# parrot-tts/Parrot-TTS

Measured on AMD Instinct MI355X. Metric: audio samples/sec (16 kHz; see config.note) + RTF, 256-unit batch-64 per GPU, higher is better.
Workload: dtype f32 (f16x3 split products)

## Files before the change

### include/parrot_hip_debug.h

```cpp
#ifndef PARROT_HIP_DEBUG_H
#define PARROT_HIP_DEBUG_H

#include "parrot_hip.h"

#ifdef __cplusplus
extern "C" {
#endif

int parrot_selftest(void* stream);
int parrot_conv_num_tile_cfgs(void);

int parrot_set_default_precision(int32_t prec);
int parrot_set_fused_resblocks(int32_t mode);
int parrot_set_tte_merge(int32_t on);
int parrot_debug_copy(const float* src, float* dst, size_t n, void* stream);
int parrot_debug_mfma_ceiling(int32_t shape, int32_t constant_data, double* tflops_out);
int parrot_prof_begin(void);
int parrot_prof_begin_row(int32_t row);
int parrot_prof_end(double* out, int32_t n_cfg);

int parrot_voc_debug_absmax(parrot_voc_t*, float* dst_dev);
int parrot_tte_debug_stages(parrot_tte_t*, float* const* enc_ptrs, float* const* dec_ptrs);
size_t parrot_debug_attention_workspace_bytes(int32_t B, int32_t T, int32_t H, int32_t core);
int parrot_debug_attention(const float* qkv, const uint8_t* valid, float* ctx, int32_t B, int32_t T, int32_t H, int32_t hd, int32_t core,
                           void* ws, size_t ws_bytes, void* stream);
int parrot_debug_layernorm(const float* x, const float* gamma, const float* beta, float* y, int32_t B, int32_t C, int32_t T,
                           int32_t relu_in, void* stream);
#define PARROT_DEBUG_MAX_DIM (1 << 20)
int parrot_debug_durations(const float* ld_raw, const uint8_t* src_valid, const int32_t* src_len, int32_t B, int32_t S, float* log_dur,
                           int64_t* dur, int32_t* cum, int32_t* out_len, int32_t* status, void* stream);
// ... 60 lines not shown
```

### parrot_tts_amd/_lib.py

```python
from __future__ import annotations

import ctypes as C
import os

HERE = os.path.dirname(os.path.abspath(__file__))
LIB_PATH = os.environ.get("PARROT_HIP_LIB") or os.path.join(HERE, "libparrot_hip.so")

MAX_STAGES, MAX_KERNELS, MAX_DIL = 8, 4, 4
ABI_VERSION = 7
c_float_p = C.POINTER(C.c_float)


class ParrotHipError(RuntimeError):
    def __init__(self, code: int, msg: str):
        super().__init__(f"libparrot_hip error {code}: {msg}")
        self.code = code


class ConvDesc(C.Structure):
    _fields_ = [("c_in", C.c_int32), ("c_out", C.c_int32), ("k", C.c_int32), ("dilation", C.c_int32),
                ("padding", C.c_int32), ("transposed", C.c_int32), ("stride", C.c_int32), ("pre_act", C.c_int32),
                ("pre_slope", C.c_float), ("act", C.c_int32), ("tile_cfg", C.c_int32), ("precision", C.c_int32)]


# ... 100 lines not shown

vp, i32, sz, f32 = C.c_void_p, C.c_int32, C.c_size_t, C.c_float
SIGNATURES = {
    "parrot_abi_version": (C.c_int, []),
    "parrot_last_error": (C.c_char_p, []),
    "parrot_selftest": (C.c_int, [vp]),
    "parrot_set_default_precision": (C.c_int, [i32]),
    "parrot_set_fused_resblocks": (C.c_int, [i32]),
    "parrot_set_tte_merge": (C.c_int, [i32]),
    "parrot_conv_create": (C.c_int, [C.POINTER(vp), C.POINTER(ConvDesc), c_float_p, c_float_p]),
    "parrot_conv_destroy": (None, [vp]),
    "parrot_conv_run": (C.c_int, [vp, vp, vp, vp, i32, i32, i32, f32, vp]),
    "parrot_conv_out_len": (C.c_int, [vp, i32]),
    "parrot_conv_num_tile_cfgs": (C.c_int, []),
    "parrot_debug_copy": (C.c_int, [vp, vp, sz, vp]),
    "parrot_debug_mfma_ceiling": (C.c_int, [i32, i32, C.POINTER(C.c_double)]),
    "parrot_prof_begin": (C.c_int, []),
    "parrot_prof_begin_row": (C.c_int, [i32]),
    "parrot_prof_end": (C.c_int, [C.POINTER(C.c_double), i32]),
    "parrot_voc_create": (C.c_int, [C.POINTER(vp), C.POINTER(VocCfg), C.POINTER(VocWeights)]),
    "parrot_voc_create_ex": (C.c_int, [C.POINTER(vp), C.POINTER(VocCfg), C.POINTER(VocWeights), i32, i32]),
    "parrot_voc_destroy": (None, [vp]),
    "parrot_voc_precision": (C.c_int, [vp]),
    "parrot_voc_debug_absmax": (C.c_int, [vp, vp]),
    "parrot_voc_workspace_bytes": (sz, [vp, i32, i32]),
    "parrot_voc_forward": (C.c_int, [vp, vp, vp, vp, i32, i32, vp, C.POINTER(vp), vp, sz, vp]),
    "parrot_voc_forward_feats": (C.c_int, [vp, vp, vp, vp, i32, vp, i32, i32, vp, C.POINTER(vp), vp, sz, vp]),
    "parrot_voc_chunked_workspace_bytes": (sz, [vp, i32, i32, i32]),
    "parrot_voc_forward_chunked": (C.c_int, [vp, vp, vp, vp, i32, i32, i32, i32, vp, vp, sz, vp]),
    "parrot_voc_check": (C.c_int, [vp, vp]),
# ... 131 lines not shown
```

### parrot_tts_amd/csrc/conv_mfma.h

```cpp
#pragma once
#include <hip/hip_runtime.h>
#include <stdint.h>
#include <algorithm>

#include "conv_consts.h"
#include "div_uniform.h"

namespace parrot {

__host__ __device__ __forceinline__ int row_true_len(int n, int mul, int add) { return n > 0 ? n * mul + add : 0; }

struct DynLdsOnce {
    bool done[64] = {};
};
inline hipError_t ensure_dyn_lds(DynLdsOnce& st, const void* kern, size_t lds) {
    int dev = 0;
    hipError_t e = hipGetDevice(&dev);
    if (e != hipSuccess) return e;
    const bool tracked = dev >= 0 && dev < 64;
    if (tracked && st.done[dev]) return hipSuccess;
    e = hipFuncSetAttribute(kern, hipFuncAttributeMaxDynamicSharedMemorySize, (int)lds);
    if (e == hipSuccess && tracked) st.done[dev] = true;
    return e;
}
// ... 23 lines not shown
    int act;
    int epi;
    float div;
    int u;
    int tiles_n;
    long x_bstride;
    long y_bstride;
    long res_bstride;
    int groups;
    int Mg;
    int u_inv16;
    const int32_t* row_len;
    int row_len_mul;
    int row_len_add;
    int fold_res;
    int lean;
    int n_cus;
    int epi16;
    float acc_scale;
    float out_scale;
    const void* xplane;
    void* yplane;
    long xplane_bstride;
    long yplane_bstride;
    float yplane_slope;
    int plane_only;
};

__device__ __forceinline__ float apply_act(float v, int act) { return (act == ACT_RELU && v < 0.f) ? 0.f : v; }

// ... 146 lines not shown
#pragma unroll
                    for (int q = 0; q < 8; ++q) yv[q] = yb[off[q] < 0 ? 0 : off[q]];
                }
                float v[8];
#pragma unroll
                for (int q = 0; q < 8; ++q) v[q] = yv[q] + (fmaxf(acc[mt][nt][g * 8 + q], act_lo) + rv[q]);
                if (do_div) div_rows(dv, v);
#pragma unroll
                for (int q = 0; q < 8; ++q)
                    if (off[q] >= 0) yb[off[q]] = v[q];
            }
        }
    }
}

struct RowTile {
    __amdgpu_buffer_rsrc_t rsrc;
};
__device__ __forceinline__ RowTile row_tile(const float* base, int rows, int row_elems) {
    const size_t a = reinterpret_cast<size_t>(base);
    const unsigned lo = __builtin_amdgcn_readfirstlane((unsigned)a), hi = __builtin_amdgcn_readfirstlane((unsigned)(a >> 32));
    RowTile t;
    t.rsrc = __builtin_amdgcn_make_buffer_rsrc(reinterpret_cast<void*>(((size_t)hi << 32) | lo), 0,
                                               __builtin_amdgcn_readfirstlane(rows * row_elems * 4), 0x00020000);
    return t;
}
__device__ __forceinline__ float row_tile_load(const RowTile& t, int voff, int soff) {
    return __builtin_bit_cast(float, __builtin_amdgcn_raw_buffer_load_b32(t.rsrc, voff, soff, 0));
}
__device__ __forceinline__ void row_tile_store(const RowTile& t, float v, int voff, int soff) {
// ... 272 lines not shown
```

### parrot_tts_amd/csrc/conv_split.h

```cpp
#pragma once
#include <cstdlib>
#include <type_traits>

#include "conv_mfma.h"

namespace parrot {

typedef short s16x8 __attribute__((ext_vector_type(8)));
typedef __bf16 bf16x8 __attribute__((ext_vector_type(8)));
typedef _Float16 f16x8 __attribute__((ext_vector_type(8)));

typedef __bf16 bf16x2 __attribute__((ext_vector_type(2)));
typedef _Float16 f16x2 __attribute__((ext_vector_type(2)));
typedef float f32x2 __attribute__((ext_vector_type(2)));
__device__ __forceinline__ unsigned pk_bf16(float x0, float x1) {
    const f32x2 v = {x0, x1};
    return __builtin_bit_cast(unsigned, __builtin_convertvector(v, bf16x2));
}
__device__ __forceinline__ unsigned pk_f16(float x0, float x1) {
    const f32x2 v = {x0, x1};
    return __builtin_bit_cast(unsigned, __builtin_convertvector(v, f16x2));
}
__device__ __forceinline__ float max_nc(float a, float b) {
    float r;
// ... 63 lines not shown
}
template <class SCH>
__device__ __forceinline__ float pre_scale(float v, float slope) {
    if constexpr (SCH::XS != 1.f) return max_nc(v * SCH::XS, v * (SCH::XS * slope));
    else return max_nc(v, v * slope);
}

template <int N, class F>
__device__ __forceinline__ void static_for(F&& f) {
    if constexpr (N > 0) {
        static_for<N - 1>(f);
        f(std::integral_constant<int, N - 1>{});
    }
}

template <class SCH, int WAVES_M, int WAVES_N, int WM, int WN, int MINW, int K, int SUBS = 1, bool LEAN = false>
__global__ __launch_bounds__(WAVES_M* WAVES_N * 64, MINW) void conv_split_kernel(const ConvParams p) {
    static_assert(SUBS == 1 || K == 1, "sub-slab staging: 1x1 convs only (no halo)");
    constexpr int NPC = SCH::NP, NTERM = SCH::NT;
    constexpr int NW = WAVES_M * WAVES_N, NT = NW * 64;
    constexpr int BM = WAVES_M * WM * 32;
    constexpr int BN = WAVES_N * WN * 32;
    constexpr int COLS = BN + ((SUBS > 1 && K == 1) ? 0 : CONV_HALO);
    constexpr int PIECE_BYTES = COLS * 32;
    constexpr int SUB_BYTES = NPC * PIECE_BYTES;
    constexpr int BUF_BYTES = SUBS * SUB_BYTES;
    constexpr int LIVE = SUBS * COLS * 2;
    constexpr int ITEMS = (LIVE + NT - 1) / NT;
    constexpr int KS = K * SUBS;
    constexpr int STEP_BYTES = NPC * 1024;

    extern __shared__ __attribute__((aligned(16))) char smem_raw[];

    const int tid = threadIdx.x;
    const int lane = tid & 63;
    const int wave = __builtin_amdgcn_readfirstlane(tid >> 6);
    const int wm = wave / WAVES_N;
    const int wn = wave % WAVES_N;
    const int half = lane >> 5;
    const int l31 = lane & 31;

    const int n_mb = (p.M + BM - 1) / BM;
    const int n_tiles = p.tiles_n * p.B, tpx = (n_tiles + 7) >> 3;
    const int xcd = blockIdx.x & 7, seq = blockIdx.x >> 3;
// ... 70 lines not shown
    for (int mt = 0; mt < WM; ++mt)
        abase[mt] = __builtin_amdgcn_readfirstlane((int)((mblock * (BM / 32) + wm * WM + mt) * p.n_it * STEP_BYTES));
    const unsigned lane16 = lane * 16;
    const int nsup = p.nchunks / SUBS;
    const int colbase = wn * WN * 32 + l31;
    auto load_b = [&](s16x8 (&bb)[WN][NPC], const char* __restrict__ xs, int tap) {
        const int col = colbase + tap * p.dil;
        const int off = col * 32 + ((half ^ ((col >> 3) & 1)) * 16);
#pragma unroll
        for (int nt = 0; nt < WN; ++nt)
#pragma unroll
            for (int pc = 0; pc < NPC; ++pc) bb[nt][pc] = *reinterpret_cast<const s16x8*>(xs + pc * PIECE_BYTES + nt * 1024 + off);
    };
    constexpr int TM = WM * WN, NMF = NTERM * TM;
    if constexpr (K > 0) {
        s16x8 A[2][WM][NPC], Bv[2][WN][NPC];
        auto load_a_piece = [&](s16x8 (&a)[WM][NPC], int pc, int soff) {
#pragma unroll
            for (int mt = 0; mt < WM; ++mt)
                a[mt][pc] = __builtin_bit_cast(s16x8, __builtin_amdgcn_raw_buffer_load_b128(wrsrc, lane16 + pc * 1024, abase[mt] + soff, 0));
        };
        auto next_chunk = [&](int q) { return (q + 1 == nsup) ? 0 : q + 1; };
        int cc = 0, cn = next_chunk(0);
#pragma unroll
        for (int pc = 0; pc < NPC; ++pc) {
            load_a_piece(A[0], pc, cc * KS * STEP_BYTES);
            load_a_piece(A[1], pc, (KS > 1 ? cc * KS + 1 : cn * KS) * STEP_BYTES);
        }
        load_slab(0);
        store_slab(0);
        __syncthreads();
        auto chunk = [&](auto par, int c) __attribute__((always_inline)) {
            constexpr int PAR = decltype(par)::value;
            const char* __restrict__ xs = smem_raw + (c & 1) * BUF_BYTES;
            const int cn2 = next_chunk(cn);
            load_slab(cn);
            load_b(Bv[PAR], xs, 0);
#pragma unroll
            for (int j = 0; j < KS; ++j) {
                const int cur = (PAR + j) & 1;
                const int tq = (j + 2 < KS) ? cc : (KS == 1 ? cn2 : cn);
                const int tj = (j + 2 < KS) ? j + 2 : (KS == 1 ? 0 : j + 2 - KS);
                const int soff = (tq * KS + tj) * STEP_BYTES;
                if (j + 1 < KS) load_b(Bv[cur ^ 1], xs + ((j + 1) / K) * SUB_BYTES, (j + 1) % K);
#pragma unroll
                for (int t = 0; t < NTERM; ++t) {
#pragma unroll
                    for (int mt = 0; mt < WM; ++mt)
#pragma unroll
                        for (int nt = 0; nt < WN; ++nt)
                            acc[mt][nt] = mfma32<SCH>(A[cur][mt][SCH::pa(t)], Bv[cur][nt][SCH::pb(t)], acc[mt][nt]);
#pragma unroll
                    for (int pc = 0; pc < NPC; ++pc)
                        if (t == SCH::last_a(pc)) load_a_piece(A[cur], pc, soff);
                }
            }
            constexpr int DS_START = (NPC >= 2) ? (SCH::last_a(NPC - 1) + 1) * TM - 1 + WM : 0;
            constexpr int SLAB_START = (NPC >= 2) ? (SCH::last_a(1) + 1) * TM - 1 + WM : 0;
            constexpr int SLAB_SLOTS = (NMF - SLAB_START) > 0 ? (NMF - SLAB_START) : 1, SLAB_PER = (ITEMS * 8 + SLAB_SLOTS - 1) / SLAB_SLOTS;
#pragma unroll
            for (int i = 0; i < NPC * WN; ++i) __builtin_amdgcn_sched_group_barrier(0x100, 1, 0);
#pragma unroll
            for (int j = 0; j < KS; ++j) {
                int ds_left = (j + 1 < KS) ? NPC * WN : 0, slab_left = (j == 0) ? ITEMS * 8 : 0;
#pragma unroll
                for (int m = 0; m < NMF; ++m) {
                    __builtin_amdgcn_sched_group_barrier(0x008, 1, 0);
#pragma unroll
                    for (int pc = NPC - 1; pc >= 1; --pc)
                        if (m >= (SCH::last_a(pc) + 1) * TM - 1 && m < (SCH::last_a(pc) + 1) * TM - 1 + WM) __builtin_amdgcn_sched_group_barrier(0x020, 1, 0);
                    if (m >= DS_START && ds_left > 0) {
                        __builtin_amdgcn_sched_group_barrier(0x100, 1, 0);
                        --ds_left;
                    }
                    if (m >= SLAB_START)
#pragma unroll
// ... 70 lines not shown
                xs = smem_raw + (c & 1) * BUF_BYTES;
                cc = cn;
                cn = (cc + 1 == p.nchunks) ? 0 : cc + 1;
                j = 0;
            } else {
                ++j;
            }
        };
        const int total = p.nchunks * p.k;
        for (int st = 0; st < total; st += 2) {
            step(a0, b0, a1, b1);
            if (st + 1 < total) step(a1, b1, a0, b0);
        }
    }
    if constexpr (LEAN) conv_epilogue_lean<WM, WN>(p, acc, b, m_wave, n_wave, half, l31);
    else conv_epilogue<WM, WN>(p, acc, b, m_wave, n_wave, half, l31);
}

template <class SCH, int WAVES_M, int WAVES_N, int WM, int WN, int MINW, int K, int SUBS = 1, bool LEAN = false>
inline hipError_t launch_conv_split_t(const ConvParams& p, dim3 grid, hipStream_t s) {
    constexpr int BN = WAVES_N * WN * 32;
    const size_t lds = (size_t)2 * SUBS * SCH::NP * (BN + ((SUBS > 1 && K == 1) ? 0 : CONV_HALO)) * 32;
    auto kern = conv_split_kernel<SCH, WAVES_M, WAVES_N, WM, WN, MINW, K, SUBS, LEAN>;
    static DynLdsOnce lds_once;
    {
        hipError_t e = ensure_dyn_lds(lds_once, reinterpret_cast<const void*>(kern), (size_t)lds);
        if (e != hipSuccess) return e;
    }
    hipLaunchKernelGGL(kern, grid, dim3(WAVES_M * WAVES_N * 64), lds, s, p);
    return hipGetLastError();
}

inline void split_tile(int variant, int& bm, int& bn) {
    if (variant == 2) { bm = 128; bn = 64; return; }
    if (variant == 3) { bm = 32; bn = 512; return; }
    bm = (variant & 1) ? 64 : 128;
    bn = (variant & 1) ? 256 : 128;
}
inline unsigned split_grid(const ConvParams& p, int bm) {
    const unsigned tiles = (unsigned)p.tiles_n * p.B, n_mb = (p.M + bm - 1) / bm;
    return (tiles + 7) / 8 * 8 * n_mb;
}
template <class SCH>
inline hipError_t launch_conv_split_s(int variant, const ConvParams& p, hipStream_t s) {
    int bm, bn;
    split_tile(variant, bm, bn);
    dim3 grid(split_grid(p, bm));
    if (variant == 3) return p.k == 3 ? launch_conv_split_t<SCH, 1, 4, 1, 4, 2, 3>(p, grid, s) : launch_conv_split_t<SCH, 1, 4, 1, 4, 2, 0>(p, grid, s);
    const bool lean = conv_lean_ok(p);
    if constexpr (SCH::ID == SchF16x3::ID) if (variant == 2) {
        if (p.k == 1 && p.nchunks % 4 == 0)
            return lean ? launch_conv_split_t<SCH, 4, 1, 1, 2, 3, 1, 4, true>(p, grid, s) : launch_conv_split_t<SCH, 4, 1, 1, 2, 3, 1, 4>(p, grid, s);
        switch (p.k) {
            case 1: return launch_conv_split_t<SCH, 4, 1, 1, 2, 3, 1>(p, grid, s);
            case 3: return launch_conv_split_t<SCH, 4, 1, 1, 2, 3, 3>(p, grid, s);
            case 9: return launch_conv_split_t<SCH, 4, 1, 1, 2, 3, 9>(p, grid, s);
            default: return launch_conv_split_t<SCH, 4, 1, 1, 2, 3, 0>(p, grid, s);
        }
    }
    if constexpr (SCH::ID != SchF16x3::ID) if (variant == 2) {
        if (p.k == 1 && p.nchunks % 4 == 0)
            return lean ? launch_conv_split_t<SCH, 2, 2, 2, 1, 3, 1, 4, true>(p, grid, s) : launch_conv_split_t<SCH, 2, 2, 2, 1, 3, 1, 4>(p, grid, s);
// ... 13 lines not shown
        }
    switch (p.k) {
        case 3:
            return lean ? launch_conv_split_t<SCH, 2, 2, 2, 2, 2, 3, 1, true>(p, grid, s) : launch_conv_split_t<SCH, 2, 2, 2, 2, 2, 3>(p, grid, s);
        case 7: return launch_conv_split_t<SCH, 2, 2, 2, 2, 2, 7>(p, grid, s);
        case 9: return launch_conv_split_t<SCH, 2, 2, 2, 2, 2, 9>(p, grid, s);
        case 11: return launch_conv_split_t<SCH, 2, 2, 2, 2, 2, 11>(p, grid, s);
        default: return launch_conv_split_t<SCH, 2, 2, 2, 2, 2, 0>(p, grid, s);
    }
}
template <class SCH>
inline hipError_t launch_conv_split_generic(int variant, const ConvParams& p, hipStream_t s) {
    int bm, bn;
    split_tile(variant, bm, bn);
    dim3 grid(split_grid(p, bm));
    if (variant == 3) return launch_conv_split_t<SCH, 1, 4, 1, 4, 2, 0>(p, grid, s);
    if (variant == 2) {
        if (p.k == 1 && p.nchunks % 4 == 0) return launch_conv_split_t<SCH, 2, 2, 2, 1, 3, 1, 4>(p, grid, s);
        return launch_conv_split_t<SCH, 2, 2, 2, 1, 3, 0>(p, grid, s);
    }
    if (variant & 1) return launch_conv_split_t<SCH, 1, 4, 2, 2, 2, 0>(p, grid, s);
    return launch_conv_split_t<SCH, 2, 2, 2, 2, 2, 0>(p, grid, s);
}
hipError_t launch_conv_split_f16x3(int variant, const ConvParams& p, hipStream_t s);
hipError_t launch_conv_split_bf16x6(int variant, const ConvParams& p, hipStream_t s);
hipError_t launch_conv_split_bf16(int variant, const ConvParams& p, hipStream_t s);
hipError_t launch_conv_split_f16(int variant, const ConvParams& p, hipStream_t s);
inline hipError_t launch_conv_split(int scheme, int variant, const ConvParams& p, hipStream_t s) {
    switch (scheme) {
        case SchBf16x6::ID: return launch_conv_split_bf16x6(variant, p, s);
// ... 9 lines not shown
```

### parrot_tts_amd/csrc/host_common.h

```cpp
#pragma once
#include "../../include/parrot_hip_debug.h"

#include <hip/hip_runtime.h>

#include <memory>
#include <string>

#include "conv_consts.h"

namespace parrot {

int fail(int code, const std::string& msg);
}
#define HIP_TRY(expr)                                                                              \
    do {                                                                                           \
        hipError_t _e = (expr);                                                                    \
        if (_e != hipSuccess)                                                                      \
            return fail(PARROT_E_HIP, std::string(#expr) + ": " + hipGetErrorString(_e));          \
    } while (0)
#define TRY(expr)                \
    do {                         \
        int _r = (expr);         \
        if (_r != PARROT_OK) return _r; \
    } while (0)
// ... 79 lines not shown

}

struct parrot_conv {
    parrot_conv_desc d{};
    int groups = 1;
    int M = 0, Mg = 0, Cout = 0, Cin = 0;
    int kk = 1, dil = 1, pad_left = 0, u = 1;
    int cfg = 0;
    int nchunks = 0, n_it = 0;
    float* wfrag = nullptr;
    float* bias = nullptr;
    int prec = 0;
    uint16_t* wfrag16 = nullptr;
    int n_it16 = 0;
    float wscale = 1.f;
    bool mfma16 = false;
    int* err_flag = nullptr;
    bool late_res = false;
    int valu_kind = 0;
    float* wraw = nullptr;

    ~parrot_conv() {
        if (wraw) (void)hipFree(wraw);
        if (wfrag16) (void)hipFree(wfrag16);
        if (wfrag) (void)hipFree(wfrag);
        if (bias) (void)hipFree(bias);
    }
    int out_len(int Tin) const {
        if (!d.transposed) return Tin + 2 * d.padding - d.dilation * (d.k - 1);
// ... 32 lines not shown
```

### parrot_tts_amd/csrc/host_conv.hip

```cpp
#include "host_common.h"

#include <algorithm>
#include <cstdio>
#include <cstring>
#include <vector>

#include "conv_split.h"
#include "conv_split16.h"
#include "conv_mfma16.h"
#include "conv_valu.h"
#include "kernels_conv.h"
#include "weight_pack.h"

using namespace parrot;
static_assert(SchBf16x6::ID == PARROT_PREC_BF16X6 && SchF16x3::ID == PARROT_PREC_F16X3 && SchBf16::ID == PARROT_PREC_BF16 && SchF16::ID == PARROT_PREC_F16,
              "weight_pack.h reads a scheme off its PARROT_PREC_* number");

static int choose_cfg(int M, int k) {
    if (M <= 16) return 6;
    if (M <= 32) return 2;
    if (M <= 64) return 1;
    return (k <= 3) ? 3 : 0;
}

static bool valu_kernels_enabled() {
    static const bool on = [] { const char* e = getenv("PARROT_VALU_KERNELS"); return !e || atoi(e) != 0; }();
    return on;
}
static bool mfma16_enabled() {
    static const bool on = [] { const char* e = getenv("PARROT_MFMA16"); return !e || atoi(e) != 0; }();
    return on;
}
static int small_tiles_mode() {
    static const int m = [] { const char* e = getenv("PARROT_SMALL_TILES"); return e ? atoi(e) : 2; }();
    return m;
}

int parrot::conv_build(parrot_conv** out, const parrot_conv_desc* d, int groups, const float* w, const float* bias, bool allow16) {
    if (!out || !d || !w) return fail(PARROT_E_INVALID, "conv_create: null argument");
    if (d->c_in <= 0 || d->c_out <= 0 || d->k <= 0 || d->dilation <= 0 || groups <= 0 || d->c_in % groups || d->c_out % groups)
        return fail(PARROT_E_INVALID, "conv_create: bad dimensions");
    std::unique_ptr<parrot_conv> c(new parrot_conv());
    c->d = *d;
    c->groups = groups;
    c->Cout = d->c_out;
    c->Cin = d->c_in / groups;
    int dmin = 0;
    if (d->transposed) {
        if (d->stride > 64) return fail(PARROT_E_UNSUPPORTED, "conv_create: transposed stride > 64");
        if (groups != 1 || d->dilation != 1 || d->stride <= 0) return fail(PARROT_E_UNSUPPORTED, "conv_create: transposed conv needs groups=1, dilation=1");
        const int u = d->stride, p = d->padding, k = d->k;
        int dlo = 1 << 30, dhi = -(1 << 30);
        for (int r = 0; r < u; ++r)
            for (int kap = 0; kap < k; ++kap)
                if ((r + p - kap) % u == 0) {
                    int dl = (r + p - kap) / u;
                    dlo = std::min(dlo, dl);
                    dhi = std::max(dhi, dl);
                }
        if (dlo > dhi) return fail(PARROT_E_INVALID, "conv_create: transposed conv has no taps");
        dmin = dlo;
        c->u = u;
        c->kk = dhi - dlo + 1;
        c->dil = 1;
        c->pad_left = -dlo;
        c->M = d->c_out * u;
    } else {
        if (d->stride > 1) return fail(PARROT_E_UNSUPPORTED, "conv_create: strided Conv1d is not on the path");
        c->u = 1;
        c->kk = d->k;
        c->dil = d->dilation;
        c->pad_left = d->padding;
        c->M = d->c_out;
    }
// ... 18 lines not shown
    if (want_prec >= 1 && c->Mg >= 32 && d->tile_cfg < 0 && c->Cin % 16 == 0 && slope_ok) {
        c->prec = want_prec;
        c->cfg = (c->Mg <= 32) ? 2 : (c->Mg <= 64) ? 1 : 0;
        const TileCfg t16 = tile_cfg(c->cfg);
        if (groups > 1 && c->Mg % t16.bm) return fail(PARROT_E_UNSUPPORTED, "conv_create: rows per group must be a multiple of the tile height");
        if (scheme_is_f16(want_prec)) c->wscale = f16_weight_scale(w, (size_t)d->c_in / groups * d->c_out * d->k);
        c->mfma16 = allow16 && mfma16_enabled() && split16_has(want_prec, c->kk) && !d->transposed && groups == 1 && c->Cin % 32 == 0 && c->M >= 64;
        int rows = 32, bm = t16.bm;
        if (c->mfma16) {
            int bn16;
            rows = 16;
            split16_tile(c->M >= 128 ? 0 : 1, bm, bn16);
        }
        const int chans = 512 / rows;
        c->nchunks = (c->Cin + chans - 1) / chans;
        c->n_it16 = c->nchunks * c->kk;
        const size_t n_steps = (size_t)((c->M + bm - 1) / bm * (bm / rows)) * c->n_it16;
        const size_t n16 = (n_steps + 1) * scheme_pieces(want_prec) * 512;
        if (n16 * sizeof(uint16_t) >= ((size_t)1 << 31)) return fail(PARROT_E_UNSUPPORTED, "conv_create: packed weight stream larger than 2 GiB");
        std::vector<uint16_t> pk16(n16, 0);
        const int n_it16 = c->n_it16;
        pack_pieces(pk16.data(), n_steps, want_prec, c->wscale, W, [=](size_t st, int lane, int e) {
            const int mt = (int)(st / n_it16), ch = (int)(st % n_it16) / kk, j = (int)(st % n_it16) % kk;
            return WeightAt{mt * rows + lane % rows, ch * chans + 8 * (lane / rows) + e, j};
        });
        HIP_TRY(hipMalloc((void**)&c->wfrag16, pk16.size() * sizeof(uint16_t)));
        HIP_TRY(hipMemcpy(c->wfrag16, pk16.data(), pk16.size() * sizeof(uint16_t), hipMemcpyHostToDevice));
    } else {
        const size_t n_steps = c->cfg == 6 ? (size_t)c->n_it : (size_t)((c->M + t.bm - 1) / t.bm * (t.bm / 32)) * c->n_it;
        std::vector<float> pk((n_steps + 1) * 256, 0.f);
        if (c->cfg == 6)
            pack_f32(pk.data(), n_steps, W, [=](size_t st, int lane, int e) { return WeightAt{lane & 15, (int)st / kk * 16 + 4 * e + (lane >> 4), (int)st % kk}; });
        else {
            const int n_it = c->n_it;
            pack_f32(pk.data(), n_steps, W, [=](size_t st, int lane, int e) {
                const int mt = (int)(st / n_it), r = (int)(st % n_it), q = r % QN, j = r / QN % kk, ch = r / QN / kk;
                return WeightAt{mt * 32 + (lane & 31), ch * CI + 8 * q + 2 * e + (lane >> 5), j};
            });
        }
// ... 48 lines not shown
    ConvParams p{};
    p.x = x; p.wfrag = c->wfrag; p.bias = c->bias; p.res = res; p.y = y;
    p.B = B; p.Cin = c->Cin; p.Tin = Tin; p.M = c->M; p.Cout = c->Cout;
    p.Ncols = (c->u > 1) ? (Tout + c->u - 1) / c->u : Tout;
    p.Tout = Tout;
    p.k = c->kk; p.dil = c->dil; p.pad_left = c->pad_left;
    p.nchunks = c->nchunks; p.n_it = c->n_it;
    p.pre = c->d.pre_act; p.pre_slope = c->d.pre_slope; p.act = c->d.act;
    p.epi = epi; p.div = div; p.u = c->u; p.u_inv16 = (65536 + c->u - 1) / c->u;
    p.groups = c->groups; p.Mg = c->Mg;
    p.row_len = o.rows.len; p.row_len_mul = o.rows.mul; p.row_len_add = o.rows.add;
    p.acc_scale = p.out_scale = 1.f;
    p.lean = 1;
    p.n_cus = num_cus();
    p.fold_res = c->late_res ? 0 : 1;
    if (pl.xplane || pl.yplane) {
        if (!plane_ok(c) || (pl.yplane && epi != EPI_STORE)) return fail(PARROT_E_INVALID, "conv_run: operand planes need a conv_split16 layer (k = 7 / 11) and EPI_STORE");
        p.xplane = pl.xplane; p.yplane = pl.yplane;
        p.xplane_bstride = (long)plane_row_bytes(c->prec, c->Cin, Tin);
        p.yplane_bstride = (long)plane_row_bytes(c->prec, c->M, Tout);
        p.yplane_slope = pl.yslope; p.plane_only = pl.plane_only;
    }
    p.x_bstride = (long)c->d.c_in * Tin;
    p.y_bstride = (long)c->Cout * Tout;
    p.res_bstride = p.y_bstride;
    int cfg = c->cfg;
    if (c->prec == 0 && (cfg == 0 || cfg == 3) && p.Ncols <= 64 && tile_cfg(4).ci == tile_cfg(cfg).ci) cfg = 4;
    if (c->prec >= 1) {
        p.wfrag = reinterpret_cast<const float*>(c->wfrag16);
        p.n_it = c->n_it16;
// ... 63 lines not shown
extern "C" int parrot_conv_create(parrot_conv_t** out, const parrot_conv_desc* d, const float* w_host, const float* bias_host) {
    return conv_build(out, d, 1, w_host, bias_host);
}
extern "C" void parrot_conv_destroy(parrot_conv_t* c) { delete c; }
extern "C" int parrot_conv_out_len(const parrot_conv_t* c, int32_t T_in) { return c ? c->out_len(T_in) : PARROT_E_INVALID; }
extern "C" int parrot_conv_num_tile_cfgs(void) { return NUM_TILE_CFGS; }
extern "C" int parrot_conv_run(parrot_conv_t* c, const float* x, const float* res, float* y, int32_t B, int32_t T_in,
                               int32_t epilogue, float div, void* stream) {
    if (!c || !x || !y) return fail(PARROT_E_INVALID, "conv_run: null argument");
    if (epilogue < 0 || epilogue > 2) return fail(PARROT_E_INVALID, "conv_run: bad epilogue");
    if (epilogue == EPI_STORE && y != x && y != res && c->out_len(T_in) > 0)
        TRY(poison(y, (size_t)B * c->Cout * c->out_len(T_in) * sizeof(float), (hipStream_t)stream));
    return conv_launch(c, x, res, y, B, T_in, epilogue, div, (hipStream_t)stream);
}

extern "C" int parrot_selftest(void* stream) {
    float* d = nullptr;
    HIP_TRY(hipMalloc((void**)&d, 64 * 16 * sizeof(float)));
    hipLaunchKernelGGL(mfma_probe_kernel, dim3(1), dim3(64), 0, (hipStream_t)stream, d);
    std::vector<float> h(64 * 16);
    hipError_t e = hipMemcpy(h.data(), d, h.size() * sizeof(float), hipMemcpyDeviceToHost);
    (void)hipFree(d);
    if (e != hipSuccess) return fail(PARROT_E_HIP, hipGetErrorString(e));
    for (int lane = 0; lane < 64; ++lane)
        for (int r = 0; r < 16; ++r) {
            const int row = (r & 3) + 8 * (r >> 2) + 4 * (lane >> 5), col = lane & 31;
            const float want = (float)(col + 1) * (float)(1001 * row + 100000);
            if (h[lane * 16 + r] != want) {
                char buf[160];
                snprintf(buf, sizeof buf, "mfma 32x32x2 layout probe: lane %d reg %d got %g want %g", lane, r, h[lane * 16 + r], want);
// ... 6 lines not shown
```

### parrot_tts_amd/csrc/weight_pack.h

```cpp
#pragma once
#include <stdint.h>

#include <algorithm>
#include <cmath>
#include <cstring>
#include <vector>

#include "../../include/parrot_hip.h"

namespace parrot {

inline int scheme_pieces(int scheme) { return scheme == PARROT_PREC_BF16X6 ? 3 : scheme == PARROT_PREC_F16X3 ? 2 : 1; }
inline bool scheme_is_f16(int scheme) { return scheme == PARROT_PREC_F16X3 || scheme == PARROT_PREC_F16; }
inline float scheme_xs(int scheme) { return scheme_is_f16(scheme) ? 8.f : 1.f; }

inline uint16_t f16_rn_host(float x) {
    const _Float16 h = (_Float16)x;
    uint16_t u;
    memcpy(&u, &h, 2);
    return u;
}
inline float f16_to_f(uint16_t u) {
    _Float16 h;
    memcpy(&h, &u, 2);
// ... 43 lines not shown
    int c_out, u, padding, dmin;
    float operator()(int m, int i, int j) const {
        if (m >= M || i >= Cin) return 0.f;
        if (transposed) {
            const int o = m / u, r = m % u;
            const int kap = r + padding - (j + dmin) * u;
            return (kap >= 0 && kap < k) ? w[((size_t)i * c_out + o) * k + kap] : 0.f;
        }
        return j < k ? w[((size_t)m * Cin + i) * k + j] : 0.f;
    }
};
struct WeightAt {
    int m, i, j;
};

struct ChainGroups { int G, Mg; };
inline ChainGroups chain_groups(int scheme, int cin, int rows) {
    int G = 1;
    if (scheme == PARROT_PREC_F32)
        for (int g = 8; g > 1 && G == 1; --g)
            if (cin % (16 * g) == 0) G = g;
    return {G, G > 1 ? (rows + 127) / 128 * 128 : rows};
}

template <typename Layout>
inline void pack_f32(float* dst, size_t n_steps, const GemmWeights& W, Layout at) {
    for (size_t st = 0; st < n_steps; ++st)
        for (int lane = 0; lane < 64; ++lane)
            for (int e = 0; e < 4; ++e) {
                const WeightAt q = at(st, lane, e);
// ... 20 lines not shown
```

Baseline: 308.4 million.

## Group transposed-conv output phases so each M tile runs only two of three taps

For stride-2/4 transposed convs with three gather offsets, output rows are regrouped by phase so each 32-row tile only needs two of the three input shifts. The packed weight stream keeps two steps per chunk instead of three, and a new kernel variant loads three B fragments and indexes taps by tile parity, with a dedicated epilogue that scatters permuted rows back to interleaved output positions. This removes MFMA work on weight taps that are structurally zero. In exchange it adds complexity: a permuted row mapping, a different epilogue store pattern, and extra B-register pressure. A debug entry point is added to inspect the step lists.

```diff
diff --git a/include/parrot_hip_debug.h b/include/parrot_hip_debug.h
--- a/include/parrot_hip_debug.h
+++ b/include/parrot_hip_debug.h
@@ -14,6 +14,8 @@
 int parrot_set_fused_resblocks(int32_t mode);
 int parrot_set_tte_merge(int32_t on);
 int parrot_debug_copy(const float* src, float* dst, size_t n, void* stream);
+int parrot_debug_convt_steps(const parrot_conv_desc* d, const float* w_host, int32_t steps_on, int32_t* info, int32_t* row_map,
+                             uint8_t* kept, uint8_t* nonzero);
 int parrot_debug_mfma_ceiling(int32_t shape, int32_t constant_data, double* tflops_out);
 int parrot_prof_begin(void);
 int parrot_prof_begin_row(int32_t row);
diff --git a/parrot_tts_amd/_lib.py b/parrot_tts_amd/_lib.py
--- a/parrot_tts_amd/_lib.py
+++ b/parrot_tts_amd/_lib.py
@@ -138,6 +138,8 @@
     "parrot_conv_out_len": (C.c_int, [vp, i32]),
     "parrot_conv_num_tile_cfgs": (C.c_int, []),
     "parrot_debug_copy": (C.c_int, [vp, vp, sz, vp]),
+    "parrot_debug_convt_steps": (C.c_int, [C.POINTER(ConvDesc), c_float_p, i32, C.POINTER(i32), C.POINTER(i32), C.POINTER(C.c_uint8),
+                                           C.POINTER(C.c_uint8)]),
     "parrot_debug_mfma_ceiling": (C.c_int, [i32, i32, C.POINTER(C.c_double)]),
     "parrot_prof_begin": (C.c_int, []),
     "parrot_prof_begin_row": (C.c_int, [i32]),
diff --git a/parrot_tts_amd/csrc/conv_mfma.h b/parrot_tts_amd/csrc/conv_mfma.h
--- a/parrot_tts_amd/csrc/conv_mfma.h
+++ b/parrot_tts_amd/csrc/conv_mfma.h
@@ -61,6 +61,7 @@
     int row_len_mul;
     int row_len_add;
     int fold_res;
+    int convt_steps;
     int lean;
     int n_cus;
     int epi16;
@@ -237,6 +238,65 @@
     }
 }
 
+template <int WM, int WN>
+__device__ __forceinline__ void conv_epilogue_steps(const ConvParams& p, f32x16 (&acc)[WM][WN], int b, int m_wave, int n_wave, int half,
+                                                    int l31) {
+    static_assert(WM == 1 || WM == 2, "one tile or one tile pair per wave");
+    typedef float f32x2_t __attribute__((ext_vector_type(2)));
+    float* __restrict__ yb = p.y + (size_t)b * p.y_bstride;
+    if (p.out_scale != 1.f) {
+#pragma unroll
+        for (int mt = 0; mt < WM; ++mt)
+#pragma unroll
+            for (int nt = 0; nt < WN; ++nt)
+#pragma unroll
+                for (int r = 0; r < 16; ++r) acc[mt][nt][r] *= p.out_scale;
+    }
+    const int pair = m_wave >> 6, g = (m_wave >> 5) & 1;
+#pragma unroll
+    for (int nt = 0; nt < WN; ++nt) {
+        const int n = n_wave + nt * 32 + l31;
+        if (p.u == 4) {
+#pragma unroll
+            for (int q = 0; q < 4; ++q)
+#pragma unroll
+                for (int i = 0; i < 2; ++i) {
+                    const int o = pair * 16 + 4 * q + 2 * half + i, r0 = 4 * q + 2 * i;
+                    const bool ok = o < p.Cout && n < p.Ncols;
+                    const float bs = (p.bias && ok) ? p.bias[o] : 0.f;
+                    if constexpr (WM == 2) {
+                        f32x4 v;
+                        v[0] = apply_act(acc[0][nt][r0] + bs, p.act);
+                        v[1] = apply_act(acc[0][nt][r0 + 1] + bs, p.act);
+                        v[2] = apply_act(acc[1][nt][r0] + bs, p.act);
+                        v[3] = apply_act(acc[1][nt][r0 + 1] + bs, p.act);
+                        if (ok) *reinterpret_cast<f32x4*>(yb + (size_t)o * p.Tout + 4 * n) = v;
+                    } else {
+                        f32x2_t v;
+                        v[0] = apply_act(acc[0][nt][r0] + bs, p.act);
+                        v[1] = apply_act(acc[0][nt][r0 + 1] + bs, p.act);
+                        if (ok) *reinterpret_cast<f32x2_t*>(yb + (size_t)o * p.Tout + 4 * n + 2 * g) = v;
+                    }
+                }
+        } else {
+#pragma unroll
+            for (int r = 0; r < 16; ++r) {
+                const int o = pair * 32 + (r & 3) + 8 * (r >> 2) + 4 * half;
+                const bool ok = o < p.Cout && n < p.Ncols;
+                const float bs = (p.bias && ok) ? p.bias[o] : 0.f;
+                if constexpr (WM == 2) {
+                    f32x2_t v;
+                    v[0] = apply_act(acc[0][nt][r] + bs, p.act);
+                    v[1] = apply_act(acc[1][nt][r] + bs, p.act);
+                    if (ok) *reinterpret_cast<f32x2_t*>(yb + (size_t)o * p.Tout + 2 * n) = v;
+                } else {
+                    if (ok) yb[(size_t)o * p.Tout + 2 * n + g] = apply_act(acc[0][nt][r] + bs, p.act);
+                }
+            }
+        }
+    }
+}
+
 struct RowTile {
     __amdgpu_buffer_rsrc_t rsrc;
 };
diff --git a/parrot_tts_amd/csrc/conv_split.h b/parrot_tts_amd/csrc/conv_split.h
--- a/parrot_tts_amd/csrc/conv_split.h
+++ b/parrot_tts_amd/csrc/conv_split.h
@@ -101,9 +101,10 @@
     }
 }
 
-template <class SCH, int WAVES_M, int WAVES_N, int WM, int WN, int MINW, int K, int SUBS = 1, bool LEAN = false>
+template <class SCH, int WAVES_M, int WAVES_N, int WM, int WN, int MINW, int K, int SUBS = 1, bool LEAN = false, bool TS = false>
 __global__ __launch_bounds__(WAVES_M* WAVES_N * 64, MINW) void conv_split_kernel(const ConvParams p) {
     static_assert(SUBS == 1 || K == 1, "sub-slab staging: 1x1 convs only (no halo)");
+    static_assert(!TS || (K == 3 && SUBS == 1 && !LEAN && WM <= 2), "phase-grouped transposed plans: three gather offsets");
     constexpr int NPC = SCH::NP, NTERM = SCH::NT;
     constexpr int NW = WAVES_M * WAVES_N, NT = NW * 64;
     constexpr int BM = WAVES_M * WM * 32;
@@ -114,7 +115,7 @@
     constexpr int BUF_BYTES = SUBS * SUB_BYTES;
     constexpr int LIVE = SUBS * COLS * 2;
     constexpr int ITEMS = (LIVE + NT - 1) / NT;
-    constexpr int KS = K * SUBS;
+    constexpr int KS = TS ? 2 : K * SUBS;
     constexpr int STEP_BYTES = NPC * 1024;
 
     extern __shared__ __attribute__((aligned(16))) char smem_raw[];
@@ -215,7 +216,8 @@
     };
     constexpr int TM = WM * WN, NMF = NTERM * TM;
     if constexpr (K > 0) {
-        s16x8 A[2][WM][NPC], Bv[2][WN][NPC];
+        s16x8 A[2][WM][NPC], Bv[TS ? WM + 1 : 2][WN][NPC];
+        const int tapw = TS ? ((mblock * (BM / 32) + wm * WM) & 1) : 0;
         auto load_a_piece = [&](s16x8 (&a)[WM][NPC], int pc, int soff) {
 #pragma unroll
             for (int mt = 0; mt < WM; ++mt)
@@ -236,21 +238,24 @@
             const char* __restrict__ xs = smem_raw + (c & 1) * BUF_BYTES;
             const int cn2 = next_chunk(cn);
             load_slab(cn);
-            load_b(Bv[PAR], xs, 0);
+            if constexpr (TS) static_for<WM>([&](auto ic) { load_b(Bv[decltype(ic)::value], xs, tapw + decltype(ic)::value); });
+            else load_b(Bv[PAR], xs, 0);
 #pragma unroll
             for (int j = 0; j < KS; ++j) {
                 const int cur = (PAR + j) & 1;
                 const int tq = (j + 2 < KS) ? cc : (KS == 1 ? cn2 : cn);
                 const int tj = (j + 2 < KS) ? j + 2 : (KS == 1 ? 0 : j + 2 - KS);
                 const int soff = (tq * KS + tj) * STEP_BYTES;
-                if (j + 1 < KS) load_b(Bv[cur ^ 1], xs + ((j + 1) / K) * SUB_BYTES, (j + 1) % K);
+                if constexpr (TS) {
+                    if (j == 0) load_b(Bv[WM], xs, tapw + WM);
+                } else if (j + 1 < KS) load_b(Bv[cur ^ 1], xs + ((j + 1) / K) * SUB_BYTES, (j + 1) % K);
 #pragma unroll
                 for (int t = 0; t < NTERM; ++t) {
 #pragma unroll
                     for (int mt = 0; mt < WM; ++mt)
 #pragma unroll
                         for (int nt = 0; nt < WN; ++nt)
-                            acc[mt][nt] = mfma32<SCH>(A[cur][mt][SCH::pa(t)], Bv[cur][nt][SCH::pb(t)], acc[mt][nt]);
+                            acc[mt][nt] = mfma32<SCH>(A[cur][mt][SCH::pa(t)], Bv[TS ? j + mt : cur][nt][SCH::pb(t)], acc[mt][nt]);
 #pragma unroll
                     for (int pc = 0; pc < NPC; ++pc)
                         if (t == SCH::last_a(pc)) load_a_piece(A[cur], pc, soff);
@@ -260,7 +265,7 @@
             constexpr int SLAB_START = (NPC >= 2) ? (SCH::last_a(1) + 1) * TM - 1 + WM : 0;
             constexpr int SLAB_SLOTS = (NMF - SLAB_START) > 0 ? (NMF - SLAB_START) : 1, SLAB_PER = (ITEMS * 8 + SLAB_SLOTS - 1) / SLAB_SLOTS;
 #pragma unroll
-            for (int i = 0; i < NPC * WN; ++i) __builtin_amdgcn_sched_group_barrier(0x100, 1, 0);
+            for (int i = 0; i < NPC * WN * (TS ? WM : 1); ++i) __builtin_amdgcn_sched_group_barrier(0x100, 1, 0);
 #pragma unroll
             for (int j = 0; j < KS; ++j) {
                 int ds_left = (j + 1 < KS) ? NPC * WN : 0, slab_left = (j == 0) ? ITEMS * 8 : 0;
@@ -361,14 +366,15 @@
         }
     }
     if constexpr (LEAN) conv_epilogue_lean<WM, WN>(p, acc, b, m_wave, n_wave, half, l31);
+    else if constexpr (TS) conv_epilogue_steps<WM, WN>(p, acc, b, m_wave, n_wave, half, l31);
     else conv_epilogue<WM, WN>(p, acc, b, m_wave, n_wave, half, l31);
 }
 
-template <class SCH, int WAVES_M, int WAVES_N, int WM, int WN, int MINW, int K, int SUBS = 1, bool LEAN = false>
+template <class SCH, int WAVES_M, int WAVES_N, int WM, int WN, int MINW, int K, int SUBS = 1, bool LEAN = false, bool TS = false>
 inline hipError_t launch_conv_split_t(const ConvParams& p, dim3 grid, hipStream_t s) {
     constexpr int BN = WAVES_N * WN * 32;
     const size_t lds = (size_t)2 * SUBS * SCH::NP * (BN + ((SUBS > 1 && K == 1) ? 0 : CONV_HALO)) * 32;
-    auto kern = conv_split_kernel<SCH, WAVES_M, WAVES_N, WM, WN, MINW, K, SUBS, LEAN>;
+    auto kern = conv_split_kernel<SCH, WAVES_M, WAVES_N, WM, WN, MINW, K, SUBS, LEAN, TS>;
     static DynLdsOnce lds_once;
     {
         hipError_t e = ensure_dyn_lds(lds_once, reinterpret_cast<const void*>(kern), (size_t)lds);
@@ -389,10 +395,19 @@
     return (tiles + 7) / 8 * 8 * n_mb;
 }
 template <class SCH>
+inline hipError_t launch_conv_split_steps(int variant, const ConvParams& p, dim3 grid, hipStream_t s) {
+    if (p.k != 3 || variant > 2) return hipErrorInvalidValue;
+    if (variant == 1) return launch_conv_split_t<SCH, 1, 4, 2, 2, 2, 3, 1, false, true>(p, grid, s);
+    if (variant == 0) return launch_conv_split_t<SCH, 2, 2, 2, 2, 2, 3, 1, false, true>(p, grid, s);
+    if constexpr (SCH::ID == SchF16x3::ID) return launch_conv_split_t<SCH, 4, 1, 1, 2, 3, 3, 1, false, true>(p, grid, s);
+    else return launch_conv_split_t<SCH, 2, 2, 2, 1, 3, 3, 1, false, true>(p, grid, s);
+}
+template <class SCH>
 inline hipError_t launch_conv_split_s(int variant, const ConvParams& p, hipStream_t s) {
     int bm, bn;
     split_tile(variant, bm, bn);
     dim3 grid(split_grid(p, bm));
+    if (p.convt_steps) return launch_conv_split_steps<SCH>(variant, p, grid, s);
     if (variant == 3) return p.k == 3 ? launch_conv_split_t<SCH, 1, 4, 1, 4, 2, 3>(p, grid, s) : launch_conv_split_t<SCH, 1, 4, 1, 4, 2, 0>(p, grid, s);
     const bool lean = conv_lean_ok(p);
     if constexpr (SCH::ID == SchF16x3::ID) if (variant == 2) {
@@ -436,6 +451,7 @@
     int bm, bn;
     split_tile(variant, bm, bn);
     dim3 grid(split_grid(p, bm));
+    if (p.convt_steps) return launch_conv_split_steps<SCH>(variant, p, grid, s);
     if (variant == 3) return launch_conv_split_t<SCH, 1, 4, 1, 4, 2, 0>(p, grid, s);
     if (variant == 2) {
         if (p.k == 1 && p.nchunks % 4 == 0) return launch_conv_split_t<SCH, 2, 2, 2, 1, 3, 1, 4>(p, grid, s);
diff --git a/parrot_tts_amd/csrc/host_common.h b/parrot_tts_amd/csrc/host_common.h
--- a/parrot_tts_amd/csrc/host_common.h
+++ b/parrot_tts_amd/csrc/host_common.h
@@ -117,6 +117,7 @@
     int prec = 0;
     uint16_t* wfrag16 = nullptr;
     int n_it16 = 0;
+    bool convt_steps = false;
     float wscale = 1.f;
     bool mfma16 = false;
     int* err_flag = nullptr;
diff --git a/parrot_tts_amd/csrc/host_conv.hip b/parrot_tts_amd/csrc/host_conv.hip
--- a/parrot_tts_amd/csrc/host_conv.hip
+++ b/parrot_tts_amd/csrc/host_conv.hip
@@ -30,6 +30,10 @@
 static bool mfma16_enabled() {
     static const bool on = [] { const char* e = getenv("PARROT_MFMA16"); return !e || atoi(e) != 0; }();
     return on;
+}
+static bool convt_steps_enabled() {
+    const char* e = getenv("PARROT_CONVT_STEPS");
+    return !e || atoi(e) != 0;
 }
 static int small_tiles_mode() {
     static const int m = [] { const char* e = getenv("PARROT_SMALL_TILES"); return e ? atoi(e) : 2; }();
@@ -46,18 +50,13 @@
     c->Cout = d->c_out;
     c->Cin = d->c_in / groups;
     int dmin = 0;
+    ConvtGeom geom;
     if (d->transposed) {
         if (d->stride > 64) return fail(PARROT_E_UNSUPPORTED, "conv_create: transposed stride > 64");
         if (groups != 1 || d->dilation != 1 || d->stride <= 0) return fail(PARROT_E_UNSUPPORTED, "conv_create: transposed conv needs groups=1, dilation=1");
-        const int u = d->stride, p = d->padding, k = d->k;
-        int dlo = 1 << 30, dhi = -(1 << 30);
-        for (int r = 0; r < u; ++r)
-            for (int kap = 0; kap < k; ++kap)
-                if ((r + p - kap) % u == 0) {
-                    int dl = (r + p - kap) / u;
-                    dlo = std::min(dlo, dl);
-                    dhi = std::max(dhi, dl);
-                }
+        const int u = d->stride;
+        geom = convt_geom(d->k, u, d->padding);
+        const int dlo = geom.dlo, dhi = geom.dhi;
         if (dlo > dhi) return fail(PARROT_E_INVALID, "conv_create: transposed conv has no taps");
         dmin = dlo;
         c->u = u;
@@ -106,15 +105,18 @@
         }
         const int chans = 512 / rows;
         c->nchunks = (c->Cin + chans - 1) / chans;
-        c->n_it16 = c->nchunks * c->kk;
+        const ConvtRows R = (d->transposed && convt_steps_enabled()) ? convt_rows(d->k, c->u, d->padding, d->c_out, geom) : ConvtRows{};
+        c->convt_steps = R.on;
+        c->n_it16 = c->nchunks * (R.on ? ConvtRows::STEPS : c->kk);
         const size_t n_steps = (size_t)((c->M + bm - 1) / bm * (bm / rows)) * c->n_it16;
         const size_t n16 = (n_steps + 1) * scheme_pieces(want_prec) * 512;
         if (n16 * sizeof(uint16_t) >= ((size_t)1 << 31)) return fail(PARROT_E_UNSUPPORTED, "conv_create: packed weight stream larger than 2 GiB");
         std::vector<uint16_t> pk16(n16, 0);
         const int n_it16 = c->n_it16;
         pack_pieces(pk16.data(), n_steps, want_prec, c->wscale, W, [=](size_t st, int lane, int e) {
-            const int mt = (int)(st / n_it16), ch = (int)(st % n_it16) / kk, j = (int)(st % n_it16) % kk;
-            return WeightAt{mt * rows + lane % rows, ch * chans + 8 * (lane / rows) + e, j};
+            const int mt = (int)(st / n_it16), spc = R.on ? ConvtRows::STEPS : kk, ch = (int)(st % n_it16) / spc;
+            const int j = (int)(st % n_it16) % spc + (R.on ? ConvtRows::first_tap(mt) : 0);
+            return WeightAt{R.row(mt * rows + lane % rows), ch * chans + 8 * (lane / rows) + e, j};
         });
         HIP_TRY(hipMalloc((void**)&c->wfrag16, pk16.size() * sizeof(uint16_t)));
         HIP_TRY(hipMemcpy(c->wfrag16, pk16.data(), pk16.size() * sizeof(uint16_t), hipMemcpyHostToDevice));
@@ -193,6 +195,7 @@
     p.lean = 1;
     p.n_cus = num_cus();
     p.fold_res = c->late_res ? 0 : 1;
+    p.convt_steps = c->convt_steps ? 1 : 0;
     if (pl.xplane || pl.yplane) {
         if (!plane_ok(c) || (pl.yplane && epi != EPI_STORE)) return fail(PARROT_E_INVALID, "conv_run: operand planes need a conv_split16 layer (k = 7 / 11) and EPI_STORE");
         p.xplane = pl.xplane; p.yplane = pl.yplane;
@@ -286,6 +289,43 @@
     return conv_launch(c, x, res, y, B, T_in, epilogue, div, (hipStream_t)stream);
 }
 
+extern "C" int parrot_debug_convt_steps(const parrot_conv_desc* d, const float* w_host, int32_t steps_on, int32_t* info, int32_t* row_map,
+                                        uint8_t* kept, uint8_t* nonzero) {
+    if (!d || !info) return fail(PARROT_E_INVALID, "debug_convt_steps: null argument");
+    if (!d->transposed || d->c_in <= 0 || d->c_out <= 0 || d->k <= 0 || d->stride <= 0 || d->stride > 64 || d->c_in % 16)
+        return fail(PARROT_E_INVALID, "debug_convt_steps: a transposed conv with c_in % 16 == 0");
+    const ConvtGeom geom = convt_geom(d->k, d->stride, d->padding);
+    if (geom.dlo > geom.dhi) return fail(PARROT_E_INVALID, "debug_convt_steps: transposed conv has no taps");
+    const int u = d->stride, kk = geom.dhi - geom.dlo + 1, M = d->c_out * u, n_tiles = (M + 31) / 32, nchunks = d->c_in / 16;
+    const bool on = steps_on < 0 ? convt_steps_enabled() : steps_on != 0;
+    const ConvtRows R = on ? convt_rows(d->k, u, d->padding, d->c_out, geom) : ConvtRows{};
+    info[0] = M; info[1] = n_tiles; info[2] = nchunks; info[3] = kk; info[4] = R.on ? 1 : 0; info[5] = geom.dlo;
+    if (row_map)
+        for (int m = 0; m < M; ++m) row_map[m] = R.row(m);
+    if (!kept && !nonzero) return PARROT_OK;
+    if (!w_host) return fail(PARROT_E_INVALID, "debug_convt_steps: the step lists need the weights");
+    const int scheme = d->precision >= 1 ? d->precision : PARROT_PREC_F16X3;
+    if (scheme > PARROT_PREC_F16) return fail(PARROT_E_INVALID, "debug_convt_steps: unknown precision");
+    const float wscale = scheme_is_f16(scheme) ? f16_weight_scale(w_host, (size_t)d->c_in * d->c_out * d->k) : 1.f;
+    const GemmWeights W{w_host, M, d->c_in, d->k, true, d->c_out, u, d->padding, geom.dlo};
+    for (int t = 0; t < n_tiles; ++t)
+        for (int ch = 0; ch < nchunks; ++ch)
+            for (int j = 0; j < kk; ++j) {
+                const size_t at = ((size_t)t * nchunks + ch) * kk + j;
+                if (kept) kept[at] = !R.on || (j >= ConvtRows::first_tap(t) && j < ConvtRows::first_tap(t) + ConvtRows::STEPS);
+                if (!nonzero) continue;
+                bool nz = false;
+                for (int l = 0; l < 32 && !nz; ++l)
+                    for (int i = 0; i < 16 && !nz; ++i) {
+                        uint16_t h[3];
+                        split_weight(W(R.row(t * 32 + l), ch * 16 + i, j), scheme, wscale, h);
+                        nz = ((h[0] | h[1] | h[2]) & 0x7fff) != 0;
+                    }
+                nonzero[at] = nz;
+            }
+    return PARROT_OK;
+}
+
 extern "C" int parrot_selftest(void* stream) {
     float* d = nullptr;
     HIP_TRY(hipMalloc((void**)&d, 64 * 16 * sizeof(float)));
diff --git a/parrot_tts_amd/csrc/weight_pack.h b/parrot_tts_amd/csrc/weight_pack.h
--- a/parrot_tts_amd/csrc/weight_pack.h
+++ b/parrot_tts_amd/csrc/weight_pack.h
@@ -81,6 +81,46 @@
     int m, i, j;
 };
 
+struct ConvtGeom {
+    int dlo = 1 << 30, dhi = -(1 << 30);
+    uint32_t mask[64] = {};
+};
+inline ConvtGeom convt_geom(int k, int u, int p) {
+    ConvtGeom g;
+    for (int r = 0; r < u && r < 64; ++r)
+        for (int kap = 0; kap < k; ++kap)
+            if ((r + p - kap) % u == 0) {
+                g.dlo = std::min(g.dlo, (r + p - kap) / u);
+                g.dhi = std::max(g.dhi, (r + p - kap) / u);
+            }
+    for (int r = 0; r < u && r < 64; ++r)
+        for (int kap = 0; kap < k; ++kap)
+            if ((r + p - kap) % u == 0 && (r + p - kap) / u - g.dlo < 32) g.mask[r] |= 1u << ((r + p - kap) / u - g.dlo);
+    return g;
+}
+
+struct ConvtRows {
+    bool on = false;
+    int u = 1, M = 0;
+    int row(int ms) const {
+        if (!on || ms >= M) return ms;
+        const int tile = ms >> 5, l = ms & 31, hu = u / 2;
+        return ((tile >> 1) * (64 / u) + l / hu) * u + (tile & 1) * hu + l % hu;
+    }
+    static int first_tap(int tile) { return tile & 1; }
+    static constexpr int STEPS = 2;
+};
+inline ConvtRows convt_rows(int k, int u, int p, int c_out, const ConvtGeom& g) {
+    ConvtRows R;
+    R.u = u;
+    R.M = c_out * u;
+    if ((u != 2 && u != 4) || g.dhi - g.dlo != 2 || k - 2 * p != u || c_out % (64 / u)) return R;
+    for (int r = 0; r < u; ++r)
+        if (g.mask[r] & (r < u / 2 ? 4u : 1u)) return R;
+    R.on = true;
+    return R;
+}
+
 struct ChainGroups { int G, Mg; };
 inline ChainGroups chain_groups(int scheme, int cin, int rows) {
     int G = 1;
```

Result: no change. 310.5 million, median of 6 (+0.7%).
